# AIGeeksGroup/UniVid

Measured on AMD Instinct MI355X. Metric: denoise_steps_per_sec, higher is better.
Workload: dtype bf16

## Files before the change

include/univid_hip.h:

```cpp
#ifndef UNIVID_HIP_H
#define UNIVID_HIP_H
#include <stdint.h>
#ifdef __cplusplus
extern "C" {
#endif

int uv_version(void);
const char* uv_build_id(void);
int uv_init(void);
const char* uv_last_error(void);
int uv_device_arch(char* buf, int len);
int uv_host_blocking_sync(int on);

#define UV_OPT_CONV_HALO 0
#define UV_OPT_GEMM_GM 1
#define UV_OPT_ATTN_CUT 2
int uv_set_option(int key, int value);
int uv_get_option(int key, int* value);
int uv_reset_options(void);

#define UV_EPI_BF16 0
#define UV_EPI_GELU_BF16 1
#define UV_EPI_F32_FROM_BF16 2
#define UV_EPI_RESID_F32 3
#define UV_EPI_GATE_RESID_F32 4
#define UV_EPI_BF16_T 5

int uv_gemm_bf16_nt(const void* A, long lda, const void* W, long ldw, const void* bias_bf16, int M, int N, int K,
                    int epilogue, void* out, long ldo, const float* gate, const int32_t* gate_tid, long gate_stride,
                    int tile_cfg, void* stream);

int uv_gemm_bf16_nt_ws(const void* A, long lda, const void* W, long ldw, const void* bias_bf16, int M, int N, int K,
                       int epilogue, void* out, long ldo, const float* gate, const int32_t* gate_tid, long gate_stride,
                       int tile_cfg, void* workspace, long workspace_bytes, void* stream);
long uv_gemm_splitk_ws_bytes(int M, int N, int K);

int uv_gemm_f16_nt(const void* A, long lda, const void* W, long ldw, const void* bias_f16, int M, int N, int K, int epilogue,
                   void* out, long ldo, const float* gate, const int32_t* gate_tid, long gate_stride, int tile_cfg, void* stream);

int uv_gemm_bf16_nt_ssq(const void* A, long lda, const void* W, long ldw, const void* bias_bf16, int M, int N, int K, void* out, long ldo,
                        float* ssq, long ld_ssq, int tile_cfg, void* stream);
int uv_rms_scale_from_ssq(const float* ssq, long ld_ssq, int M, int groups, int C, float eps, float* rs, void* stream);

int uv_lora_down_bf16(const void* x, long ldx, const void* A, long lda, const float* scale, int M, int K, int R, void* out, long ldo,
                      int Rpad, void* stream);


int uv_mx_quant_bf16(const void* x, long ldx, void* codes, long ldc, void* scales, long ld_s, int M, int K, void* stream);

int uv_gemm_mxfp8_nt(const void* A, long lda, const void* A_scale, long ld_as, const void* W, long ldw, const void* W_scale, long ld_ws,
// ... 101 lines not shown
```

univid_amd/_lib.py:

```python
import ctypes
import os

import torch

_HERE = os.path.dirname(os.path.abspath(__file__))
LIB_PATH = os.path.join(_HERE, "libunivid_hip.so")

_c = ctypes
_P, _L, _I, _F = _c.c_void_p, _c.c_long, _c.c_int, _c.c_float

SIGNATURES = {
    "uv_version": [],
    "uv_init": [],
    "uv_last_error": [],
    "uv_build_id": [],
    "uv_device_arch": [_c.c_char_p, _I],
    "uv_host_blocking_sync": [_I],
    "uv_set_option": [_I, _I],
    "uv_get_option": [_I, _c.POINTER(_I)],
    "uv_reset_options": [],
    "uv_gemm_bf16_nt": [_P, _L, _P, _L, _P, _I, _I, _I, _I, _P, _L, _P, _P, _L, _I, _P],
    "uv_gemm_bf16_nt_ws": [_P, _L, _P, _L, _P, _I, _I, _I, _I, _P, _L, _P, _P, _L, _I, _P, _L, _P],
    "uv_gemm_splitk_ws_bytes": [_I, _I, _I],
    "uv_gemm_f16_nt": [_P, _L, _P, _L, _P, _I, _I, _I, _I, _P, _L, _P, _P, _L, _I, _P],
    "uv_mx_quant_bf16": [_P, _L, _P, _L, _P, _L, _I, _I, _P],
    "uv_gemm_mxfp8_nt": [_P, _L, _P, _L, _P, _L, _P, _L, _P, _I, _I, _I, _I, _P, _L, _P, _P, _L, _P],
    "uv_gemm_f32_nt": [_P, _L, _P, _L, _P, _I, _I, _I, _P, _L, _P, _L, _P],
    "uv_gemm_bf16_nt_ssq": [_P, _L, _P, _L, _P, _I, _I, _I, _P, _L, _P, _L, _I, _P],
    "uv_rms_scale_from_ssq": [_P, _L, _I, _I, _I, _F, _P, _P],
    "uv_lora_down_bf16": [_P, _L, _P, _L, _P, _I, _I, _I, _P, _L, _I, _P],
    "uv_cast_f32_bf16_rows": [_P, _L, _P, _L, _I, _I, _P],
    "uv_flash_attn_bf16_qnorm": [_P, _L, _P, _L, _P, _L, _P, _L, _I, _I, _I, _I, _I, _F, _P, _P, _P],
    "uv_flash_attn_bf16": [_P, _L, _P, _L, _P, _L, _P, _L, _I, _I, _I, _I, _I, _F, _P],
    "uv_flash_attn_f16": [_P, _L, _P, _L, _P, _L, _P, _L, _I, _I, _I, _I, _I, _F, _P],
    "uv_flash_attn_kernel_name": [_I, _I, _L, _L, _I, _c.c_char_p, _I],
    "uv_flash_attn_plan": [_I, _I, _I, _I, _I, _L, _L, _I, _c.c_char_p, _I, _c.POINTER(_I), _c.POINTER(_I), _c.POINTER(_I)],
    "uv_transpose_16": [_P, _L, _P, _L, _I, _I, _I, _P],
    "uv_cast_f32_to16": [_P, _P, _L, _I, _P],
# ... 31 lines not shown
    "uv_vae_split_f16": [_P, _L, _P, _L, _L, _I, _P, _P],
    "uv_split_weights_f16x3": [_P, _P, _L, _F, _P],
    "uv_split_weights_bf16x3": [_P, _P, _L, _P],
    "uv_split_weights_bf16x6": [_P, _P, _L, _P],
    "uv_vae_rms_silu": [_P, _L, _P, _P, _L, _L, _I, _I, _I, _P],
    "uv_softmax_rows_f32": [_P, _L, _I, _I, _F, _P],
    "uv_vae_dupup_add": [_P, _P, _I, _I, _I, _I, _I, _I, _I, _P],
    "uv_vae_avgdown_add": [_P, _P, _I, _I, _I, _I, _I, _I, _I, _P],
    "uv_vae_latent_in": [_P, _P, _P, _P, _L, _I, _L, _P],
    "uv_vae_latent_out": [_P, _L, _P, _P, _P, _I, _L, _P],
    "uv_vae_video_in": [_P, _P, _L, _I, _I, _I, _I, _I, _P],
    "uv_vae_video_out": [_P, _L, _P, _I, _I, _I, _I, _I, _P],
}
_RESTYPE = {"uv_last_error": _c.c_char_p, "uv_build_id": _c.c_char_p, "uv_gemm_splitk_ws_bytes": _L}

OPT_CONV_HALO, OPT_GEMM_GM, OPT_ATTN_CUT = range(3)
EPI_BF16, EPI_GELU_BF16, EPI_F32_FROM_BF16, EPI_RESID_F32, EPI_GATE_RESID_F32, EPI_BF16_T = range(6)

_lib = None
_inited = set()


class UnividHipError(RuntimeError):
    pass


def load(path=None):
    global _lib
    if _lib is not None:
        return _lib
    path = path or LIB_PATH
    if not os.path.exists(path):
# ... 136 lines not shown
    idx = torch.cuda.current_device() if dev.index is None else dev.index
    lib = load()
    with torch.cuda.device(idx):
        if lib.uv_host_blocking_sync(1 if on else 0) != 0:
            raise UnividHipError(lib.uv_last_error().decode())


def gemm_splitk_ws_bytes(M, N, K, device=None):
    dev = torch.device("cuda" if device is None else device)
    idx = torch.cuda.current_device() if dev.index is None else dev.index
    lib = init(idx)
    with torch.cuda.device(idx):
        return int(lib.uv_gemm_splitk_ws_bytes(int(M), int(N), int(K)))


def gemm_bf16(a, w, bias, out, epi, M=None, gate=None, gate_tid=None, tile_cfg=0, ws=None):
    f16 = a.dtype == torch.float16
    _chk(a, torch.float16 if f16 else torch.bfloat16, "gemm_bf16.a")
    _chk(w, a.dtype, "gemm_bf16.w")
    M = a.shape[0] if M is None else M
    N, K = w.shape
    if ws is not None and not f16:
        _chk(ws, torch.uint8, "gemm_bf16.ws")
        call("uv_gemm_bf16_nt_ws", ptr(a), a.stride(0), ptr(w), w.stride(0), ptr(bias), M, N, K, epi, ptr(out), out.stride(0),
             ptr(gate), ptr(gate_tid), 0 if gate is None else gate.stride(0), tile_cfg, ptr(ws), ws.numel(), stream_ptr(), flops=2 * M * N * K)
        return out
    call("uv_gemm_f16_nt" if f16 else "uv_gemm_bf16_nt", ptr(a), a.stride(0), ptr(w), w.stride(0), ptr(bias), M, N, K, epi, ptr(out), out.stride(0),
         ptr(gate), ptr(gate_tid), 0 if gate is None else gate.stride(0), tile_cfg, stream_ptr(), flops=2 * M * N * K)
    return out

# ... 162 lines not shown
```

univid_amd/csrc/capi.hip:

```cpp
#include "common.h"
#include <stdarg.h>
#include <stdio.h>
#include <atomic>

static thread_local char g_err[512] = "";

void uv_set_error(const char* fmt, ...) {
    va_list ap;
    va_start(ap, fmt);
    vsnprintf(g_err, sizeof(g_err), fmt, ap);
    va_end(ap);
}

extern "C" const char* uv_last_error(void) { return g_err; }

extern "C" int uv_version(void) { return 200; }

#ifndef UV_BUILD_ID
#define UV_BUILD_ID "unstamped"
#endif
extern "C" const char* uv_build_id(void) { return UV_BUILD_ID; }

static std::atomic<int> g_opt[UV_OPT_COUNT] = {{-1}, {0}, {0}};
static const int kOptDefault[UV_OPT_COUNT] = {-1, 0, 0};
int uv_option(int key) { return g_opt[key].load(std::memory_order_relaxed); }

extern "C" int uv_set_option(int key, int value) {
    UV_CHECK_ARG(key >= 0 && key < UV_OPT_COUNT, "uv_set_option: unknown key %d", key);
    if (key == UV_OPT_CONV_HALO) UV_CHECK_ARG(value >= -1 && value <= 1, "uv_set_option(UV_OPT_CONV_HALO): value %d not in {-1, 0, 1}", value);
    if (key == UV_OPT_GEMM_GM) UV_CHECK_ARG(value >= 0 && value <= 64, "uv_set_option(UV_OPT_GEMM_GM): value %d not in 0..64", value);
    if (key == UV_OPT_ATTN_CUT) UV_CHECK_ARG(value >= 0 && value <= 4096, "uv_set_option(UV_OPT_ATTN_CUT): value %d not in 0..4096", value);
    g_opt[key].store(value, std::memory_order_relaxed);
    return 0;
}

extern "C" int uv_get_option(int key, int* value) {
    UV_CHECK_ARG(key >= 0 && key < UV_OPT_COUNT && value, "uv_get_option: unknown key %d or null result pointer", key);
    *value = uv_option(key);
    return 0;
}

extern "C" int uv_reset_options(void) {
    for (int i = 0; i < UV_OPT_COUNT; ++i) g_opt[i].store(kOptDefault[i], std::memory_order_relaxed);
    return 0;
}
// ... 37 lines not shown
```

univid_amd/csrc/common.h:

```cpp
#pragma once
#include <hip/hip_runtime.h>
#include <stdint.h>
#include <mutex>

typedef uint16_t bf16_t;

typedef __attribute__((ext_vector_type(8))) __bf16 bf16x8;
typedef __attribute__((ext_vector_type(4))) __bf16 bf16x4;
typedef __attribute__((ext_vector_type(4))) float f32x4;
typedef __attribute__((ext_vector_type(16))) float f32x16;
typedef __attribute__((ext_vector_type(4))) uint32_t u32x4;
typedef __attribute__((ext_vector_type(2))) uint32_t u32x2;

#define UV_WAVE 64

#define UV_MAX_DEV 16
static inline int uv_cur_dev() {
    int d = 0;
    (void)hipGetDevice(&d);
    return (unsigned)d < UV_MAX_DEV ? d : 0;
}
#define UV_ONCE_PER_DEVICE(...)                                                      \
    do {                                                                             \
        static std::once_flag uv_once_[UV_MAX_DEV];                                  \
// ... 68 lines not shown
__device__ __forceinline__ f32x2 gelu_tanh_f32x2(f32x2 x) {
    const f32x2 kA = {-2.3022081986f, -2.3022081986f}, kB = {-0.1029432396f, -0.1029432396f}, one = {1.0f, 1.0f};
    const f32x2 q = __builtin_elementwise_fma(x * x, kB, kA);
    const f32x2 t = x * q;
    const f32x2 e = {__builtin_amdgcn_exp2f(t[0]), __builtin_amdgcn_exp2f(t[1])};
    const f32x2 d = one + e;
    const f32x2 c = {__builtin_amdgcn_rcpf(d[0]), __builtin_amdgcn_rcpf(d[1])};
    return x * c;
}

__device__ __forceinline__ float silu_f32(float x) { return x / (1.0f + expf(-x)); }

#define UV_OPT_CONV_HALO 0
#define UV_OPT_GEMM_GM 1
#define UV_OPT_ATTN_CUT 2
#define UV_OPT_COUNT 3
int uv_option(int key);

extern "C" const char* uv_last_error(void);
void uv_set_error(const char* fmt, ...);

#define UV_CHECK_ARG(cond, ...)            \
    do {                                   \
        if (!(cond)) {                     \
            uv_set_error(__VA_ARGS__);     \
            return -1;                     \
        }                                  \
    } while (0)

#define UV_CHECK_LAUNCH(name)                                                     \
    do {                                                                          \
// ... 7 lines not shown
```

univid_amd/csrc/gemm_bf16.hip:

```cpp
#include "gemm_bf16_kernels.h"
#include <limits.h>

int uv_gemm_diag_launch(const GemmArgs& a, int epilogue, int tile_cfg, hipStream_t s);

struct GemmWs { void* p = nullptr; long bytes = 0; };

enum GemmKernel {
    GK_PERSIST,
    GK_PINGPONG,
    GK_RING128,
    GK_T128,
    GK_T256,
    GK_T256x192,
    GK_SPLITK4,
    GK_SPLITK2,
    GK_DIAG,
};
struct GemmStep { GemmKernel kernel; int m0, rows; };
struct GemmPlan { int n; GemmStep step[2]; };

static long whole_rounds_cut(int M, int N, int ncus) {
    const long tiles_n = (N + 255) / 256, tiles_m = (M + 255) / 256;
    const long rounds = tiles_m * tiles_n / ncus;
    return rounds * ncus / tiles_n * 256;
}
static long persistent_cut(int M, int N, int ncus, bool* short_round) {
    const long tiles = (long)((M + 255) / 256) * (N / 256);
    const long rounds = tiles / ncus, rest = tiles - rounds * ncus;
    *short_round = rounds >= 1 && rest > 0 && rest * 100 < 45 * ncus;
    return *short_round ? whole_rounds_cut(M, N, ncus) : (long)(M / 256) * 256;
}

static GemmPlan plan_gemm(int M, int N, int K, int epilogue, long ldo, int tile_cfg, bool F16, int ncus, long ws_bytes, bool ws_aligned) {
    auto whole = [&](GemmKernel k) { return GemmPlan{1, {{k, 0, M}}}; };
    auto cut_at = [&](long cut, GemmKernel main, GemmKernel strip) {
        return cut <= 0 || cut >= M ? whole(main) : GemmPlan{2, {{main, 0, (int)cut}, {strip, (int)cut, M - (int)cut}}};
    };
    switch (tile_cfg) {
        case 0: break;
        case 1: return whole(GK_T128);
        case 5: return whole(GK_T256);
        case 6: return whole(GK_T256x192);
        case 7: return whole(GK_PINGPONG);
        case 8: return cut_at(whole_rounds_cut(M, N, ncus), GK_PINGPONG, GK_RING128);
        case 9: return cut_at(whole_rounds_cut(M, N, ncus), GK_T256, GK_RING128);
        case 12: return whole(GK_RING128);
        case 17: return whole(GK_PERSIST);
        case 18: {
            const long tm = (long)(M / 256) * 256;
            return cut_at(tm > 0 && tm < M ? tm : whole_rounds_cut(M, N, ncus), GK_PERSIST, GK_RING128);
        }
        case 19: return whole(GK_SPLITK4);
        case 20: return whole(GK_SPLITK2);
        default: return whole(GK_DIAG);
    }
    if (M >= 2048 && N >= 1024 && N % 256 == 0 && K % 128 == 0 && K >= 384 &&
        (ldo % 8 == 0 || epilogue == UV_EPI_BF16_T || (epilogue >= UV_EPI_F32_FROM_BF16 && epilogue != UV_EPI_BF16_SSQ))) {
        bool short_round = false;
        const long cut = persistent_cut(M, N, ncus, &short_round);
        if (cut / 256 * (N / 256) < 2L * ncus || (epilogue == UV_EPI_BF16_T && ldo % 8 != 0))
            return short_round ? cut_at(whole_rounds_cut(M, N, ncus), GK_PINGPONG, GK_RING128) : whole(GK_PINGPONG);
        const int rows = M - (int)cut;
        const long strip_tiles = (long)((rows + 255) / 256) * (N / 256);
        const bool splitk = !F16 && (epilogue == UV_EPI_BF16 || epilogue == UV_EPI_RESID_F32 || epilogue == UV_EPI_GATE_RESID_F32) &&
                            K >= 8192 && K % 512 == 0 && strip_tiles * 4 <= ncus && ws_aligned && ws_bytes >= splitk_ws_bytes(rows, N, 4);
        return cut_at(cut, GK_PERSIST, splitk ? GK_SPLITK4 : GK_RING128);
    }
    if (M < 2048 || N < 1024) {
        if (M >= 4096 && N >= 512 && N % 256 == 0 && K % 128 == 0 && K >= 256 && ldo % 8 == 0 && M % 256 == 0 &&
            2L * (M / 256) * (N / 256) >= ncus)
            return whole(GK_PINGPONG);
        const long t128 = (long)((M + 127) / 128) * ((N + 127) / 128);
        return whole(t128 <= 2 * ncus ? GK_RING128 : GK_T128);
    }
    const long tm = (M + 255) / 256;
    const long t256 = tm * ((N + 255) / 256), t192 = tm * ((N + 191) / 192);
    const double c256 = (double)((t256 + 255) / 256) * 1.00, c192 = (double)((t192 + 255) / 256) * 0.78;
    return whole(!F16 && N % 192 == 0 && c192 < c256 && K <= 4096 && epilogue != UV_EPI_BF16_SSQ ? GK_T256x192 : GK_T256);
}

static GemmArgs rows_of(const GemmArgs& a, int epilogue, long m0, int rows) {
    GemmArgs r = a;
    r.M = rows;
    r.A = a.A + m0 * a.lda;
    if (a.gate_tid) r.gate_tid = a.gate_tid + m0;
    if (a.ssq) r.ssq = a.ssq + m0 * a.ld_ssq;
    if (epilogue == UV_EPI_BF16_T) r.out = (bf16_t*)a.out + m0;
    else if (epilogue == UV_EPI_BF16 || epilogue == UV_EPI_GELU_BF16 || epilogue == UV_EPI_BF16_SSQ) r.out = (bf16_t*)a.out + m0 * a.ldo;
    else r.out = (float*)a.out + m0 * a.ldo;
    return r;
}

template <bool F16>
static int launch_step(GemmKernel kernel, const GemmArgs& a, int epilogue, int tile_cfg, hipStream_t s, const GemmWs& ws) {
    switch (kernel) {
        case GK_PERSIST:
            UV_CHECK_ARG(a.K % 128 == 0 && a.K >= 384, "uv_gemm_bf16_nt: tile_cfg 17 needs K %% 128 == 0 and K >= 384 (K=%d)", a.K);
            return launch_8ph_persist<F16>(a, epilogue, s);
        case GK_PINGPONG:
            UV_CHECK_ARG(a.K % 128 == 0 && a.K >= 256, "uv_gemm_bf16_nt: tile_cfg 7 needs K %% 128 == 0 and K >= 256 (K=%d)", a.K);
            return launch_8ph<5, F16>(a, epilogue, s);
        case GK_RING128: return launch_cfg<128, 128, 4, 2, 4, F16>(a, epilogue, s);
        case GK_T128: return launch_cfg<128, 128, 2, 2, 2, F16>(a, epilogue, s);
        case GK_T256: return launch_cfg<256, 256, 4, 4, 2, F16>(a, epilogue, s);
        case GK_T256x192: if constexpr (!F16) return launch_cfg<256, 192, 4, 4>(a, epilogue, s); break;
        case GK_SPLITK4: if constexpr (!F16) return launch_8ph_splitk<4, false>(a, epilogue, s, ws.p, ws.bytes); break;
        case GK_SPLITK2: if constexpr (!F16) return launch_8ph_splitk<2, false>(a, epilogue, s, ws.p, ws.bytes); break;
        case GK_DIAG: if constexpr (!F16) return uv_gemm_diag_launch(a, epilogue, tile_cfg, s); break;
    }
    uv_set_error("uv_gemm_f16_nt: tile_cfg %d is not built for fp16 operands", tile_cfg);
    return -1;
}

// ... 6 lines not shown
    UV_CHECK_ARG(K % UV_BK == 0, "uv_gemm_bf16_nt: K=%d must be a multiple of %d", K, UV_BK);
    UV_CHECK_ARG(N % 16 == 0, "uv_gemm_bf16_nt: N=%d must be a multiple of 16", N);
    UV_CHECK_ARG(lda % 8 == 0 && ldw % 8 == 0, "uv_gemm_bf16_nt: lda/ldw must be multiples of 8 elements");
    UV_CHECK_ARG(((uintptr_t)A & 15) == 0 && ((uintptr_t)W & 15) == 0 && ((uintptr_t)out & 15) == 0,
                 "uv_gemm_bf16_nt: pointers must be 16-byte aligned");
    UV_CHECK_ARG(ldo % 4 == 0, "uv_gemm_bf16_nt: ldo must be a multiple of 4 elements");
    if (epilogue == UV_EPI_GATE_RESID_F32)
        UV_CHECK_ARG(gate && gate_stride % 4 == 0, "uv_gemm_bf16_nt: gate table required (stride %% 4 == 0)");
    GemmArgs a;
    a.A = (const bf16_t*)A; a.W = (const bf16_t*)W; a.bias = (const bf16_t*)bias_bf16;
    a.out = out; a.gate = gate; a.gate_tid = gate_tid;
    a.lda = lda; a.ldw = ldw; a.ldo = ldo; a.gate_stride = gate_stride;
    a.M = M; a.N = N; a.K = K; a.tiles_m = a.tiles_n = 0;
    a.ssq = ssq; a.ld_ssq = ld_ssq;
    a.ws_slab = nullptr; a.ws_cnt = nullptr; a.gm = 0;
    if (epilogue == UV_EPI_BF16_SSQ)
        UV_CHECK_ARG(ssq && N % 32 == 0 && ld_ssq >= N / 32 && ldo % 8 == 0, "uv_gemm_bf16_nt_ssq: needs N %% 32 == 0, ld_ssq >= N / 32, ldo %% 8 == 0 (N=%d ld_ssq=%ld ldo=%ld)", N, ld_ssq, ldo);
    a.zeros = uv_zero_page();
    UV_CHECK_ARG(a.zeros, "uv_gemm_bf16_nt: zero page missing (call uv_init)");
    const GemmPlan plan = plan_gemm(M, N, K, epilogue, ldo, tile_cfg, F16, uv_num_cus(), ws.p ? ws.bytes : 0, ((uintptr_t)ws.p & 255) == 0);
    for (int i = 0; i < plan.n; ++i) {
        const GemmStep& st = plan.step[i];
        const int rc = launch_step<F16>(st.kernel, rows_of(a, epilogue, st.m0, st.rows), epilogue, tile_cfg, (hipStream_t)stream, ws);
        if (rc) return rc;
    }
    return 0;
}

extern "C" int uv_gemm_bf16_nt(const void* A, long lda, const void* W, long ldw, const void* bias_bf16,
                               int M, int N, int K, int epilogue, void* out, long ldo,
                               const float* gate, const int32_t* gate_tid, long gate_stride,
                               int tile_cfg, void* stream) {
    return gemm_entry<false>(A, lda, W, ldw, bias_bf16, M, N, K, epilogue, out, ldo, gate, gate_tid, gate_stride, tile_cfg, stream);
}

extern "C" int uv_gemm_bf16_nt_ws(const void* A, long lda, const void* W, long ldw, const void* bias_bf16,
                                  int M, int N, int K, int epilogue, void* out, long ldo,
                                  const float* gate, const int32_t* gate_tid, long gate_stride,
                                  int tile_cfg, void* workspace, long workspace_bytes, void* stream) {
    UV_CHECK_ARG(workspace_bytes >= 0 && (workspace || workspace_bytes == 0), "uv_gemm_bf16_nt_ws: bad workspace");
    GemmWs ws;
    ws.p = workspace; ws.bytes = workspace_bytes;
    return gemm_entry<false>(A, lda, W, ldw, bias_bf16, M, N, K, epilogue, out, ldo, gate, gate_tid, gate_stride, tile_cfg, stream, nullptr, 0, ws);
}

extern "C" long uv_gemm_splitk_ws_bytes(int M, int N, int K) {
    const GemmPlan plan = plan_gemm(M, N, K, UV_EPI_RESID_F32, N, 0, false, uv_num_cus(), LONG_MAX, true);
    const GemmStep& strip = plan.step[plan.n - 1];
    return strip.kernel == GK_SPLITK4 ? splitk_ws_bytes(strip.rows, N, 4) : 0;
}

extern "C" int uv_gemm_bf16_nt_ssq(const void* A, long lda, const void* W, long ldw, const void* bias_bf16, int M, int N, int K,
                                   void* out, long ldo, float* ssq, long ld_ssq, int tile_cfg, void* stream) {
    return gemm_entry<false>(A, lda, W, ldw, bias_bf16, M, N, K, UV_EPI_BF16_SSQ, out, ldo, nullptr, nullptr, 0, tile_cfg, stream, ssq, ld_ssq);
}

extern "C" int uv_gemm_f16_nt(const void* A, long lda, const void* W, long ldw, const void* bias_f16,
                              int M, int N, int K, int epilogue, void* out, long ldo,
                              const float* gate, const int32_t* gate_tid, long gate_stride,
                              int tile_cfg, void* stream) {
    UV_CHECK_ARG(tile_cfg == 0, "uv_gemm_f16_nt: only tile_cfg 0 (automatic) is built for fp16 operands");
    return gemm_entry<true>(A, lda, W, ldw, bias_f16, M, N, K, epilogue, out, ldo, gate, gate_tid, gate_stride, tile_cfg, stream);
}
```

univid_amd/csrc/gemm_bf16_kernels.h:

```cpp
#pragma once
#include "common.h"
#include <stdlib.h>
#include <type_traits>

const float* uv_zero_page();

#define UV_BK 64

enum {
    UV_EPI_BF16 = 0,
    UV_EPI_GELU_BF16 = 1,
    UV_EPI_F32_FROM_BF16 = 2,
    UV_EPI_RESID_F32 = 3,
    UV_EPI_GATE_RESID_F32 = 4,
    UV_EPI_BF16_T = 5,
    UV_EPI_BF16_SSQ = 6,
};

struct GemmArgs {
    const bf16_t* A;
    const bf16_t* W;
    const bf16_t* bias;
    void* out;
    const float* gate;
    const int32_t* gate_tid;
    const float* zeros;
    long lda, ldw, ldo, gate_stride;
    int M, N, K;
    int tiles_m, tiles_n;
    int gm;
    float* ssq;
    long ld_ssq;
    float* ws_slab;
    int* ws_cnt;
};

typedef __attribute__((address_space(3))) void lds_void;

__device__ __forceinline__ void glds16(const void* g, lds_void* l) {
    __builtin_amdgcn_global_load_lds(g, l, 16, 0, 0);
}

template <int EPI, bool F16 = false, bool FULL = false>
__device__ __forceinline__ void epi_frag(const GemmArgs& p, int mb, int nb, const f32x4& a, int frow, int fq) {
    if (EPI != UV_EPI_BF16_T) {
        const int m = mb + frow, n = nb + 4 * fq;
        if (!FULL && (m >= p.M || n >= p.N)) return;
        float v[4];
#pragma unroll
// ... 164 lines not shown
        const int m = mb[f] + frow, n = nb[f] + 4 * fq;
        float v[4];
        v[0] = acc[f][0] + in16<F16>((bf16_t)(bb[slot][0] & 0xffff));
        v[1] = acc[f][1] + in16<F16>((bf16_t)(bb[slot][0] >> 16));
        v[2] = acc[f][2] + in16<F16>((bf16_t)(bb[slot][1] & 0xffff));
        v[3] = acc[f][3] + in16<F16>((bf16_t)(bb[slot][1] >> 16));
        f32x4 x = xb[slot];
#pragma unroll
        for (int e = 0; e < 4; ++e)
            x[e] = GATE ? __fadd_rn(x[e], __fmul_rn(round16<F16>(v[e]), gb[slot][e])) : __fadd_rn(x[e], round16<F16>(v[e]));
        if (m < p.M && n < p.N) *(f32x4*)((float*)p.out + (long)m * p.ldo + n) = x;
        if (f + D < NF) issue(f + D, slot);
    }
}

template <int BM, int BN, int WM, int WN, int EPI, int NS = 2, bool F16 = false>
__global__ __launch_bounds__(WM* WN * 64) void gemm_bf16_nt_kernel(GemmArgs p) {
    constexpr int NW = WM * WN;
    constexpr int NT = NW * 64;
    constexpr int TM = BM / WM / 16;
    constexpr int TN = BN / WN / 16;
    constexpr int A_BYTES = BM * 128;
    constexpr int W_BYTES = BN * 128;
    constexpr int STAGE_BYTES = A_BYTES + W_BYTES;
    constexpr int A_INSTR = (BM / 8 + NW - 1) / NW;
    constexpr int W_INSTR = (BN / 8 + NW - 1) / NW;
    static_assert(BM % 8 == 0 && BN % 8 == 0 && (BM / WM) % 16 == 0 && (BN / WN) % 16 == 0, "tile/wave mismatch");
    constexpr bool TRANS = (EPI == UV_EPI_BF16_T);

    extern __shared__ __attribute__((aligned(16))) char smem[];

    const int tid = threadIdx.x;
    const int lane = tid & 63;
    const int wave = __builtin_amdgcn_readfirstlane(tid >> 6);
    const int wm = wave / WN, wn = wave % WN;

    const int nblk = p.tiles_m * p.tiles_n;
    int bid = blockIdx.x;
    {
        const int q = nblk >> 3, r = nblk & 7, xcd = bid & 7, idx = bid >> 3;
        bid = (xcd < r ? xcd * (q + 1) : r * (q + 1) + (xcd - r) * q) + idx;
    }
    constexpr int GM = 4;
    const int group_sz = GM * p.tiles_n;
    const int group = bid / group_sz;
    const int first_m = group * GM;
    const int gm = min(GM, p.tiles_m - first_m);
    const int in_group = bid - group * group_sz;
    const int tile_m = first_m + in_group % gm;
    const int tile_n = in_group / gm;
    const int m0 = tile_m * BM, n0 = tile_n * BN;

    const int srow = lane >> 3;
    const int pchunk = lane & 7;
    const bf16_t* a_src[A_INSTR];
    const bf16_t* w_src[W_INSTR];
#pragma unroll
    for (int i = 0; i < A_INSTR; ++i) {
        const int row = (i * NW + wave) * 8 + srow;
        const int c = pchunk ^ ((row >> 1) & 7);
        const int gr = min(m0 + row, p.M - 1);
        a_src[i] = p.A + (long)gr * p.lda + c * 8;
    }
#pragma unroll
    for (int i = 0; i < W_INSTR; ++i) {
        const int row = (i * NW + wave) * 8 + srow;
// ... 107 lines not shown
        epi_rmw_pipe<EPI, NF, (NF >= 8 ? 4 : 2), F16>(p, mb, nb, av, frow, fq);
    } else if constexpr (EPI == UV_EPI_BF16_SSQ) {
        static_assert(TN % 2 == 0 && (BN / WN) % 32 == 0, "UV_EPI_BF16_SSQ needs whole 32-column groups per wave");
#pragma unroll
        for (int j = 0; j < TM; ++j)
#pragma unroll
            for (int i = 0; i < TN; i += 2)
                epi_pair_ssq<F16>(p, m0 + wm * (BM / WM) + j * 16, n0 + wn * (BN / WN) + i * 16, acc[i][j], acc[i + 1][j], frow, fq);
    } else {
#pragma unroll
        for (int j = 0; j < TM; ++j)
#pragma unroll
            for (int i = 0; i < TN; ++i)
                epi_frag<EPI, F16>(p, m0 + wm * (BM / WM) + j * 16, n0 + wn * (BN / WN) + i * 16, acc[i][j], frow, fq);
    }
}


template <int EPI, bool F16>
__device__ __forceinline__ void epi_rmw_rows_lds(const GemmArgs& p, char* smem, const f32x4 (&acc)[2][2][2][4], int m0, int n0,
                                                 int wave, int lane) {
    static_assert(EPI == UV_EPI_RESID_F32 || EPI == UV_EPI_GATE_RESID_F32, "rmw epilogues only");
    constexpr bool GATE = EPI == UV_EPI_GATE_RESID_F32;
    constexpr int D = 8;
    const int wr = wave >> 2, wc = wave & 3;
    const int frow = lane & 15, fq = lane >> 4;
    float bv[2][2][4];
#pragma unroll
    for (int hn = 0; hn < 2; ++hn)
#pragma unroll
// ... 314 lines not shown
                for (int hn = 0; hn < 2; ++hn)
                    epi_pair_ssq<F16>(p, m0 + hm * 128 + wr * 64 + j * 16, n0 + hn * 128 + wc * 32, acc[hn][hm][0][j], acc[hn][hm][1][j], frow, fq);
    } else {
#pragma unroll
        for (int hm = 0; hm < 2; ++hm)
#pragma unroll
            for (int j = 0; j < 4; ++j)
#pragma unroll
                for (int hn = 0; hn < 2; ++hn)
#pragma unroll
                    for (int i = 0; i < 2; ++i)
                        epi_frag<EPI, F16>(p, m0 + hm * 128 + wr * 64 + j * 16, n0 + hn * 128 + wc * 32 + i * 16, acc[hn][hm][i][j], frow, fq);
    }
}

template <int EPI, bool F16 = false>
__global__ __launch_bounds__(512) void gemm_bf16_8ph_persist_kernel(GemmArgs p) {
    constexpr bool TRANS = (EPI == UV_EPI_BF16_T);
    constexpr bool RMW = (EPI == UV_EPI_RESID_F32 || EPI == UV_EPI_GATE_RESID_F32);
    constexpr int VAR = 5;
    constexpr int HALF = 16384;
    constexpr int BUF = 4 * HALF;
    extern __shared__ __attribute__((aligned(16))) char smem[];

    const int tid = threadIdx.x;
    const int lane = tid & 63;
    const int wave = __builtin_amdgcn_readfirstlane(tid >> 6);
    const int wr = wave >> 2, wc = wave & 3;

    const int nblk = p.tiles_m * p.tiles_n;
    const int G = gridDim.x >> 3;
    int first, cnt;
    {
        const int q = nblk >> 3, r = nblk & 7, xcd = blockIdx.x & 7;
        first = xcd < r ? xcd * (q + 1) : r * (q + 1) + (xcd - r) * q;
        cnt = q + (xcd < r ? 1 : 0);
    }
    int cur = blockIdx.x >> 3;
    if (cur >= cnt) return;
    const int GM = p.gm;
    const int group_sz = GM * p.tiles_n;
    auto origin = [&](int bid, int& m0, int& n0) {
        const int group = bid / group_sz;
        const int first_m = group * GM;
        const int gm = min(GM, p.tiles_m - first_m);
        const int in_group = bid - group * group_sz;
        m0 = (first_m + in_group % gm) * 256;
        n0 = (in_group / gm) * 256;
    };
    int m0, n0;
    origin(first + cur, m0, n0);

    const int srow = lane >> 3, pchunk = lane & 7;
    const bf16_t* a_src[2][2];
// ... 90 lines not shown
                        for (int i = 0; i < 2; ++i)
                            epi_pair16_T<F16>(p, m0 + hm * 128 + wr * 64 + j * 16, n0 + hn * 128 + wc * 32 + i * 16, acc[hn][hm][i][j], acc[hn][hm][i][j + 1], frow, fq);
        } else {
#pragma unroll
            for (int hm = 0; hm < 2; ++hm)
#pragma unroll
                for (int j = 0; j < 4; ++j)
#pragma unroll
                    for (int hn = 0; hn < 2; ++hn)
#pragma unroll
                        for (int i = 0; i < 2; ++i)
                            epi_frag<EPI, F16, true>(p, m0 + hm * 128 + wr * 64 + j * 16, n0 + hn * 128 + wc * 32 + i * 16, acc[hn][hm][i][j], frow, fq);
        }
        if (!has_next) break;
        m0 = m1; n0 = n1; cur = nxt;
    }
    asm volatile("s_waitcnt vmcnt(0)" ::: "memory");
}


template <void (*KERN)(GemmArgs)>
static int launch_kernel(dim3 grid, dim3 block, size_t lds, hipStream_t stream, const GemmArgs& a, const char* who) {
    UV_ONCE_PER_DEVICE(hipFuncSetAttribute((const void*)KERN, hipFuncAttributeMaxDynamicSharedMemorySize, (int)lds));
    hipLaunchKernelGGL(KERN, grid, block, lds, stream, a);
    UV_CHECK_LAUNCH(who);
    return 0;
}

constexpr unsigned UV_EPIS_ALL = 0x7f;
constexpr bool epi_in(unsigned epis, int e) { return e >= 0 && e < 32 && (epis >> e & 1) != 0; }
// ... 40 lines not shown
    constexpr unsigned EPIS = 1u << UV_EPI_BF16 | 1u << UV_EPI_RESID_F32 | 1u << UV_EPI_GATE_RESID_F32;
    UV_CHECK_ARG(epi_in(EPIS, epi),
                 "uv_gemm_bf16_nt_ws: the split-K strip is built for the bf16 and the residual epilogues (0, 3, 4), not %d", epi);
    a.ws_cnt = (int*)ws;
    a.ws_slab = (float*)((char*)ws + 4096);
    if (hipMemsetAsync(a.ws_cnt, 0, (size_t)tiles * sizeof(int), stream) != hipSuccess) {
        uv_set_error("uv_gemm_bf16_nt_ws: hipMemsetAsync of the tile counters failed");
        return -1;
    }
    const dim3 grid(8 * ((tiles * SK + 7) / 8));
    return launch_epi<EPIS>(epi, [&](auto e) {
        return launch_kernel<gemm_bf16_8ph_kernel<decltype(e)::value, 5, F16, SK>>(grid, 512, 128 * 1024, stream, a, "uv_gemm_bf16_nt_ws");
    });
}

template <bool F16 = false>
static int launch_8ph_persist(const GemmArgs& a0, int epi, hipStream_t stream) {
    GemmArgs a = a0;
    UV_CHECK_ARG(a.M % 256 == 0 && a.N % 256 == 0, "uv_gemm_bf16_nt: the persistent kernel needs whole 256x256 tiles (M=%d N=%d)", a.M, a.N);
    UV_CHECK_ARG(a.ldo % 8 == 0 || (epi != UV_EPI_BF16_T && epi != UV_EPI_BF16 && epi != UV_EPI_GELU_BF16 && epi != UV_EPI_BF16_SSQ),
                 "uv_gemm_bf16_nt: the persistent kernel stores 16 bytes per lane: ldo=%ld must be a multiple of 8 elements", a.ldo);
    a.tiles_m = a.M / 256;
    a.tiles_n = a.N / 256;
    a.gm = (a.N <= 4096 && a.K <= 4096) ? 8 : (a.K >= 8192 ? 2 : 4);
    if (const int gm = uv_option(UV_OPT_GEMM_GM); gm > 0) a.gm = gm;
    const int tiles = a.tiles_m * a.tiles_n;
    int wgs = uv_num_cus() & ~7;
    if (wgs > tiles) wgs = tiles & ~7;
    UV_CHECK_ARG(wgs >= 8, "uv_gemm_bf16_nt: too few tiles (%d) for the persistent kernel", tiles);
    const dim3 grid(wgs);
    return launch_epi(epi, [&](auto e) {
        return launch_kernel<gemm_bf16_8ph_persist_kernel<decltype(e)::value, F16>>(grid, 512, 128 * 1024, stream, a, "uv_gemm_bf16_nt");
    });
}

template <int BM, int BN, int WM, int WN, int NS = 2, bool F16 = false>
static int launch_cfg(const GemmArgs& a0, int epi, hipStream_t stream) {
    GemmArgs a = a0;
    a.tiles_m = (a.M + BM - 1) / BM;
    a.tiles_n = (a.N + BN - 1) / BN;
    constexpr bool SSQ = (BN / WN) % 32 == 0;
    UV_CHECK_ARG(SSQ || epi != UV_EPI_BF16_SSQ, "uv_gemm_bf16_nt_ssq: this tile shape has no whole 32-column groups per wave");
    const dim3 grid(a.tiles_m * a.tiles_n);
    return launch_epi<SSQ ? UV_EPIS_ALL : UV_EPIS_ALL & ~(1u << UV_EPI_BF16_SSQ)>(epi, [&](auto e) {
        return launch_kernel<gemm_bf16_nt_kernel<BM, BN, WM, WN, decltype(e)::value, NS, F16>>(grid, WM * WN * 64, NS * (BM + BN) * 128, stream, a, "uv_gemm_bf16_nt");
    });
}
// ... 1 lines not shown
```

Measured before the change: 3.946.

## Fold the leftover row strip into the persistent GEMM kernel as 128x128 tail tiles

```diff
diff --git a/include/univid_hip.h b/include/univid_hip.h
--- a/include/univid_hip.h
+++ b/include/univid_hip.h
@@ -15,6 +15,7 @@
 #define UV_OPT_CONV_HALO 0
 #define UV_OPT_GEMM_GM 1
 #define UV_OPT_ATTN_CUT 2
+#define UV_OPT_GEMM_TAIL 3
 int uv_set_option(int key, int value);
 int uv_get_option(int key, int* value);
 int uv_reset_options(void);
@@ -34,6 +35,9 @@
                        int epilogue, void* out, long ldo, const float* gate, const int32_t* gate_tid, long gate_stride,
                        int tile_cfg, void* workspace, long workspace_bytes, void* stream);
 long uv_gemm_splitk_ws_bytes(int M, int N, int K);
+
+int uv_gemm_plan(int M, int N, int K, int epilogue, long ldo, int tile_cfg, int f16, int ncus, int* steps, int* n_steps);
+int uv_gemm_tail_tiles(int tail_rows, int N, int grid, int wg, int* tile_m, int* tile_n, int cap, int* count);
 
 int uv_gemm_f16_nt(const void* A, long lda, const void* W, long ldw, const void* bias_f16, int M, int N, int K, int epilogue,
                    void* out, long ldo, const float* gate, const int32_t* gate_tid, long gate_stride, int tile_cfg, void* stream);
diff --git a/univid_amd/_lib.py b/univid_amd/_lib.py
--- a/univid_amd/_lib.py
+++ b/univid_amd/_lib.py
@@ -22,6 +22,8 @@
     "uv_gemm_bf16_nt": [_P, _L, _P, _L, _P, _I, _I, _I, _I, _P, _L, _P, _P, _L, _I, _P],
     "uv_gemm_bf16_nt_ws": [_P, _L, _P, _L, _P, _I, _I, _I, _I, _P, _L, _P, _P, _L, _I, _P, _L, _P],
     "uv_gemm_splitk_ws_bytes": [_I, _I, _I],
+    "uv_gemm_plan": [_I, _I, _I, _I, _L, _I, _I, _I, _c.POINTER(_I), _c.POINTER(_I)],
+    "uv_gemm_tail_tiles": [_I, _I, _I, _I, _c.POINTER(_I), _c.POINTER(_I), _I, _c.POINTER(_I)],
     "uv_gemm_f16_nt": [_P, _L, _P, _L, _P, _I, _I, _I, _I, _P, _L, _P, _P, _L, _I, _P],
     "uv_mx_quant_bf16": [_P, _L, _P, _L, _P, _L, _I, _I, _P],
     "uv_gemm_mxfp8_nt": [_P, _L, _P, _L, _P, _L, _P, _L, _P, _I, _I, _I, _I, _P, _L, _P, _P, _L, _P],
@@ -83,8 +85,8 @@
 }
 _RESTYPE = {"uv_last_error": _c.c_char_p, "uv_build_id": _c.c_char_p, "uv_gemm_splitk_ws_bytes": _L}
 
-OPT_CONV_HALO, OPT_GEMM_GM, OPT_ATTN_CUT = range(3)
-EPI_BF16, EPI_GELU_BF16, EPI_F32_FROM_BF16, EPI_RESID_F32, EPI_GATE_RESID_F32, EPI_BF16_T = range(6)
+OPT_CONV_HALO, OPT_GEMM_GM, OPT_ATTN_CUT, OPT_GEMM_TAIL = range(4)
+EPI_BF16, EPI_GELU_BF16, EPI_F32_FROM_BF16, EPI_RESID_F32, EPI_GATE_RESID_F32, EPI_BF16_T, EPI_BF16_SSQ = range(7)
 
 _lib = None
 _inited = set()
@@ -251,6 +253,26 @@
         return int(lib.uv_gemm_splitk_ws_bytes(int(M), int(N), int(K)))
 
 
+GK_PERSIST, GK_PINGPONG, GK_RING128 = range(3)
+
+
+def gemm_plan(M, N, K, epi=EPI_BF16, ldo=None, tile_cfg=0, f16=False, ncus=0):
+    steps, n = (_I * 10)(), _I(0)
+    lib = load()
+    if lib.uv_gemm_plan(int(M), int(N), int(K), int(epi), int(N if ldo is None else ldo), int(tile_cfg), int(f16), int(ncus), steps, ctypes.byref(n)) != 0:
+        raise UnividHipError(lib.uv_last_error().decode())
+    return [tuple(steps[5 * i:5 * i + 5]) for i in range(n.value)]
+
+
+def gemm_tail_tiles(tail_rows, N, grid, wg):
+    cap = (tail_rows + 127) // 128 * (N // 128) + 1
+    tm, tn, n = (_I * cap)(), (_I * cap)(), _I(0)
+    lib = load()
+    if lib.uv_gemm_tail_tiles(int(tail_rows), int(N), int(grid), int(wg), tm, tn, cap, ctypes.byref(n)) != 0:
+        raise UnividHipError(lib.uv_last_error().decode())
+    return [(tm[i], tn[i]) for i in range(n.value)]
+
+
 def gemm_bf16(a, w, bias, out, epi, M=None, gate=None, gate_tid=None, tile_cfg=0, ws=None):
     f16 = a.dtype == torch.float16
     _chk(a, torch.float16 if f16 else torch.bfloat16, "gemm_bf16.a")
diff --git a/univid_amd/csrc/capi.hip b/univid_amd/csrc/capi.hip
--- a/univid_amd/csrc/capi.hip
+++ b/univid_amd/csrc/capi.hip
@@ -21,14 +21,15 @@
 #endif
 extern "C" const char* uv_build_id(void) { return UV_BUILD_ID; }
 
-static std::atomic<int> g_opt[UV_OPT_COUNT] = {{-1}, {0}, {0}};
-static const int kOptDefault[UV_OPT_COUNT] = {-1, 0, 0};
+static std::atomic<int> g_opt[UV_OPT_COUNT] = {{-1}, {0}, {0}, {0}};
+static const int kOptDefault[UV_OPT_COUNT] = {-1, 0, 0, 0};
 int uv_option(int key) { return g_opt[key].load(std::memory_order_relaxed); }
 
 extern "C" int uv_set_option(int key, int value) {
     UV_CHECK_ARG(key >= 0 && key < UV_OPT_COUNT, "uv_set_option: unknown key %d", key);
     if (key == UV_OPT_CONV_HALO) UV_CHECK_ARG(value >= -1 && value <= 1, "uv_set_option(UV_OPT_CONV_HALO): value %d not in {-1, 0, 1}", value);
     if (key == UV_OPT_GEMM_GM) UV_CHECK_ARG(value >= 0 && value <= 64, "uv_set_option(UV_OPT_GEMM_GM): value %d not in 0..64", value);
+    if (key == UV_OPT_GEMM_TAIL) UV_CHECK_ARG(value >= 0 && value <= 2, "uv_set_option(UV_OPT_GEMM_TAIL): value %d not in {0, 1, 2}", value);
     if (key == UV_OPT_ATTN_CUT) UV_CHECK_ARG(value >= 0 && value <= 4096, "uv_set_option(UV_OPT_ATTN_CUT): value %d not in 0..4096", value);
     g_opt[key].store(value, std::memory_order_relaxed);
     return 0;
diff --git a/univid_amd/csrc/common.h b/univid_amd/csrc/common.h
--- a/univid_amd/csrc/common.h
+++ b/univid_amd/csrc/common.h
@@ -106,7 +106,8 @@
 #define UV_OPT_CONV_HALO 0
 #define UV_OPT_GEMM_GM 1
 #define UV_OPT_ATTN_CUT 2
-#define UV_OPT_COUNT 3
+#define UV_OPT_GEMM_TAIL 3
+#define UV_OPT_COUNT 4
 int uv_option(int key);
 
 extern "C" const char* uv_last_error(void);
diff --git a/univid_amd/csrc/gemm_bf16.hip b/univid_amd/csrc/gemm_bf16.hip
--- a/univid_amd/csrc/gemm_bf16.hip
+++ b/univid_amd/csrc/gemm_bf16.hip
@@ -16,7 +16,7 @@
     GK_SPLITK2,
     GK_DIAG,
 };
-struct GemmStep { GemmKernel kernel; int m0, rows; };
+struct GemmStep { GemmKernel kernel; int m0, rows, tail; };
 struct GemmPlan { int n; GemmStep step[2]; };
 
 static long whole_rounds_cut(int M, int N, int ncus) {
@@ -31,10 +31,11 @@
     return *short_round ? whole_rounds_cut(M, N, ncus) : (long)(M / 256) * 256;
 }
 
-static GemmPlan plan_gemm(int M, int N, int K, int epilogue, long ldo, int tile_cfg, bool F16, int ncus, long ws_bytes, bool ws_aligned) {
-    auto whole = [&](GemmKernel k) { return GemmPlan{1, {{k, 0, M}}}; };
+static GemmPlan plan_gemm(int M, int N, int K, int epilogue, long ldo, int tile_cfg, bool F16, int ncus, long ws_bytes, bool ws_aligned,
+                          bool two_launch) {
+    auto whole = [&](GemmKernel k) { return GemmPlan{1, {{k, 0, M, 0}}}; };
     auto cut_at = [&](long cut, GemmKernel main, GemmKernel strip) {
-        return cut <= 0 || cut >= M ? whole(main) : GemmPlan{2, {{main, 0, (int)cut}, {strip, (int)cut, M - (int)cut}}};
+        return cut <= 0 || cut >= M ? whole(main) : GemmPlan{2, {{main, 0, (int)cut, 0}, {strip, (int)cut, M - (int)cut, 0}}};
     };
     switch (tile_cfg) {
         case 0: break;
@@ -64,7 +65,8 @@
         const long strip_tiles = (long)((rows + 255) / 256) * (N / 256);
         const bool splitk = !F16 && (epilogue == UV_EPI_BF16 || epilogue == UV_EPI_RESID_F32 || epilogue == UV_EPI_GATE_RESID_F32) &&
                             K >= 8192 && K % 512 == 0 && strip_tiles * 4 <= ncus && ws_aligned && ws_bytes >= splitk_ws_bytes(rows, N, 4);
-        return cut_at(cut, GK_PERSIST, splitk ? GK_SPLITK4 : GK_RING128);
+        if (splitk || two_launch || cut <= 0 || cut >= M) return cut_at(cut, GK_PERSIST, splitk ? GK_SPLITK4 : GK_RING128);
+        return GemmPlan{1, {{GK_PERSIST, 0, M, rows}}};
     }
     if (M < 2048 || N < 1024) {
         if (M >= 4096 && N >= 512 && N % 256 == 0 && K % 128 == 0 && K >= 256 && ldo % 8 == 0 && M % 256 == 0 &&
@@ -92,11 +94,11 @@
 }
 
 template <bool F16>
-static int launch_step(GemmKernel kernel, const GemmArgs& a, int epilogue, int tile_cfg, hipStream_t s, const GemmWs& ws) {
+static int launch_step(GemmKernel kernel, const GemmArgs& a, int tail, int epilogue, int tile_cfg, hipStream_t s, const GemmWs& ws) {
     switch (kernel) {
         case GK_PERSIST:
             UV_CHECK_ARG(a.K % 128 == 0 && a.K >= 384, "uv_gemm_bf16_nt: tile_cfg 17 needs K %% 128 == 0 and K >= 384 (K=%d)", a.K);
-            return launch_8ph_persist<F16>(a, epilogue, s);
+            return launch_8ph_persist<F16>(a, epilogue, s, tail);
         case GK_PINGPONG:
             UV_CHECK_ARG(a.K % 128 == 0 && a.K >= 256, "uv_gemm_bf16_nt: tile_cfg 7 needs K %% 128 == 0 and K >= 256 (K=%d)", a.K);
             return launch_8ph<5, F16>(a, epilogue, s);
@@ -133,14 +135,16 @@
     a.M = M; a.N = N; a.K = K; a.tiles_m = a.tiles_n = 0;
     a.ssq = ssq; a.ld_ssq = ld_ssq;
     a.ws_slab = nullptr; a.ws_cnt = nullptr; a.gm = 0;
+    a.tail_m0 = a.tail_rows = a.tail_fwd = 0;
     if (epilogue == UV_EPI_BF16_SSQ)
         UV_CHECK_ARG(ssq && N % 32 == 0 && ld_ssq >= N / 32 && ldo % 8 == 0, "uv_gemm_bf16_nt_ssq: needs N %% 32 == 0, ld_ssq >= N / 32, ldo %% 8 == 0 (N=%d ld_ssq=%ld ldo=%ld)", N, ld_ssq, ldo);
     a.zeros = uv_zero_page();
     UV_CHECK_ARG(a.zeros, "uv_gemm_bf16_nt: zero page missing (call uv_init)");
-    const GemmPlan plan = plan_gemm(M, N, K, epilogue, ldo, tile_cfg, F16, uv_num_cus(), ws.p ? ws.bytes : 0, ((uintptr_t)ws.p & 255) == 0);
+    const GemmPlan plan = plan_gemm(M, N, K, epilogue, ldo, tile_cfg, F16, uv_num_cus(), ws.p ? ws.bytes : 0, ((uintptr_t)ws.p & 255) == 0,
+                                    uv_option(UV_OPT_GEMM_TAIL) == 1);
     for (int i = 0; i < plan.n; ++i) {
         const GemmStep& st = plan.step[i];
-        const int rc = launch_step<F16>(st.kernel, rows_of(a, epilogue, st.m0, st.rows), epilogue, tile_cfg, (hipStream_t)stream, ws);
+        const int rc = launch_step<F16>(st.kernel, rows_of(a, epilogue, st.m0, st.rows), st.tail, epilogue, tile_cfg, (hipStream_t)stream, ws);
         if (rc) return rc;
     }
     return 0;
@@ -164,9 +168,33 @@
 }
 
 extern "C" long uv_gemm_splitk_ws_bytes(int M, int N, int K) {
-    const GemmPlan plan = plan_gemm(M, N, K, UV_EPI_RESID_F32, N, 0, false, uv_num_cus(), LONG_MAX, true);
+    const GemmPlan plan = plan_gemm(M, N, K, UV_EPI_RESID_F32, N, 0, false, uv_num_cus(), LONG_MAX, true, uv_option(UV_OPT_GEMM_TAIL) == 1);
     const GemmStep& strip = plan.step[plan.n - 1];
     return strip.kernel == GK_SPLITK4 ? splitk_ws_bytes(strip.rows, N, 4) : 0;
+}
+
+extern "C" int uv_gemm_plan(int M, int N, int K, int epilogue, long ldo, int tile_cfg, int f16, int ncus, int* steps, int* n_steps) {
+    UV_CHECK_ARG(M > 0 && N > 0 && K > 0 && ncus >= 0 && steps && n_steps, "uv_gemm_plan: bad shape M=%d N=%d K=%d, CU count %d or null result pointer", M, N, K, ncus);
+    const GemmPlan plan = plan_gemm(M, N, K, epilogue, ldo, tile_cfg, f16 != 0, ncus ? ncus : uv_num_cus(), 0, true, uv_option(UV_OPT_GEMM_TAIL) == 1);
+    for (int i = 0; i < plan.n; ++i) {
+        const GemmStep& st = plan.step[i];
+        steps[5 * i] = st.kernel; steps[5 * i + 1] = st.m0; steps[5 * i + 2] = st.rows; steps[5 * i + 3] = st.tail;
+        steps[5 * i + 4] = st.kernel == GK_PERSIST ? persist_grid(ncus ? ncus : uv_num_cus(), (long)((st.rows - st.tail) / 256) * (N / 256)) : 0;
+    }
+    *n_steps = plan.n;
+    return 0;
+}
+
+extern "C" int uv_gemm_tail_tiles(int tail_rows, int N, int grid, int wg, int* tile_m, int* tile_n, int cap, int* count) {
+    UV_CHECK_ARG(tail_rows >= 0 && N > 0 && N % 128 == 0 && grid >= 8 && grid % 8 == 0 && wg >= 0 && wg < grid && tile_m && tile_n && cap >= 0 && count,
+                 "uv_gemm_tail_tiles: bad arguments (tail_rows=%d N=%d grid=%d wg=%d)", tail_rows, N, grid, wg);
+    const int ttm = (tail_rows + 127) >> 7, ttn = N >> 7, G = grid >> 3;
+    int tfirst, tcnt, n = 0;
+    xcd_range(ttm * ttn, wg & 7, tfirst, tcnt);
+    for (int tt = tail_slot(wg >> 3, G, uv_option(UV_OPT_GEMM_TAIL) == 2); tt < tcnt; tt += G, ++n)
+        if (n < cap) walk4_tile(tfirst + tt, ttm, ttn, tile_m[n], tile_n[n]);
+    *count = n;
+    return 0;
 }
 
 extern "C" int uv_gemm_bf16_nt_ssq(const void* A, long lda, const void* W, long ldw, const void* bias_bf16, int M, int N, int K,
diff --git a/univid_amd/csrc/gemm_bf16_kernels.h b/univid_amd/csrc/gemm_bf16_kernels.h
--- a/univid_amd/csrc/gemm_bf16_kernels.h
+++ b/univid_amd/csrc/gemm_bf16_kernels.h
@@ -33,6 +33,8 @@
     long ld_ssq;
     float* ws_slab;
     int* ws_cnt;
+    int tail_m0, tail_rows;
+    int tail_fwd;
 };
 
 typedef __attribute__((address_space(3))) void lds_void;
@@ -227,8 +229,8 @@
     }
 }
 
-template <int BM, int BN, int WM, int WN, int EPI, int NS = 2, bool F16 = false>
-__global__ __launch_bounds__(WM* WN * 64) void gemm_bf16_nt_kernel(GemmArgs p) {
+template <int BM, int BN, int WM, int WN, int EPI, int NS, bool F16>
+__device__ __forceinline__ void gemm_nt_tile(const GemmArgs& p, char* smem, int m0, int n0, int tid) {
     constexpr int NW = WM * WN;
     constexpr int NT = NW * 64;
     constexpr int TM = BM / WM / 16;
@@ -241,28 +243,10 @@
     static_assert(BM % 8 == 0 && BN % 8 == 0 && (BM / WM) % 16 == 0 && (BN / WN) % 16 == 0, "tile/wave mismatch");
     constexpr bool TRANS = (EPI == UV_EPI_BF16_T);
 
-    extern __shared__ __attribute__((aligned(16))) char smem[];
-
-    const int tid = threadIdx.x;
+
     const int lane = tid & 63;
     const int wave = __builtin_amdgcn_readfirstlane(tid >> 6);
     const int wm = wave / WN, wn = wave % WN;
-
-    const int nblk = p.tiles_m * p.tiles_n;
-    int bid = blockIdx.x;
-    {
-        const int q = nblk >> 3, r = nblk & 7, xcd = bid & 7, idx = bid >> 3;
-        bid = (xcd < r ? xcd * (q + 1) : r * (q + 1) + (xcd - r) * q) + idx;
-    }
-    constexpr int GM = 4;
-    const int group_sz = GM * p.tiles_n;
-    const int group = bid / group_sz;
-    const int first_m = group * GM;
-    const int gm = min(GM, p.tiles_m - first_m);
-    const int in_group = bid - group * group_sz;
-    const int tile_m = first_m + in_group % gm;
-    const int tile_n = in_group / gm;
-    const int m0 = tile_m * BM, n0 = tile_n * BN;
 
     const int srow = lane >> 3;
     const int pchunk = lane & 7;
@@ -400,6 +384,34 @@
             for (int i = 0; i < TN; ++i)
                 epi_frag<EPI, F16>(p, m0 + wm * (BM / WM) + j * 16, n0 + wn * (BN / WN) + i * 16, acc[i][j], frow, fq);
     }
+}
+
+__host__ __device__ __forceinline__ void walk4_tile(int t, int tiles_m, int tiles_n, int& tile_m, int& tile_n) {
+    constexpr int GM = 4;
+    const int group_sz = GM * tiles_n;
+    const int group = t / group_sz;
+    const int first_m = group * GM;
+    const int gm = tiles_m - first_m < GM ? tiles_m - first_m : GM;
+    const int in_group = t - group * group_sz;
+    tile_m = first_m + in_group % gm;
+    tile_n = in_group / gm;
+}
+
+__host__ __device__ __forceinline__ void xcd_range(int n, int xcd, int& first, int& cnt) {
+    const int q = n >> 3, r = n & 7;
+    first = xcd < r ? xcd * (q + 1) : r * (q + 1) + (xcd - r) * q;
+    cnt = q + (xcd < r ? 1 : 0);
+}
+
+__host__ __device__ __forceinline__ int tail_slot(int idx, int G, int fwd) { return fwd ? idx : G - 1 - idx; }
+
+template <int BM, int BN, int WM, int WN, int EPI, int NS = 2, bool F16 = false>
+__global__ __launch_bounds__(WM* WN * 64) void gemm_bf16_nt_kernel(GemmArgs p) {
+    extern __shared__ __attribute__((aligned(16))) char smem[];
+    int first, cnt, tile_m, tile_n;
+    xcd_range(p.tiles_m * p.tiles_n, blockIdx.x & 7, first, cnt);
+    walk4_tile(first + (blockIdx.x >> 3), p.tiles_m, p.tiles_n, tile_m, tile_n);
+    gemm_nt_tile<BM, BN, WM, WN, EPI, NS, F16>(p, smem, tile_m * BM, tile_n * BN, threadIdx.x);
 }
 
 
@@ -744,7 +756,7 @@
     }
 }
 
-template <int EPI, bool F16 = false>
+template <int EPI, bool F16 = false, bool TAIL = false>
 __global__ __launch_bounds__(512) void gemm_bf16_8ph_persist_kernel(GemmArgs p) {
     constexpr bool TRANS = (EPI == UV_EPI_BF16_T);
     constexpr bool RMW = (EPI == UV_EPI_RESID_F32 || EPI == UV_EPI_GATE_RESID_F32);
@@ -758,16 +770,13 @@
     const int wave = __builtin_amdgcn_readfirstlane(tid >> 6);
     const int wr = wave >> 2, wc = wave & 3;
 
-    const int nblk = p.tiles_m * p.tiles_n;
     const int G = gridDim.x >> 3;
     int first, cnt;
-    {
-        const int q = nblk >> 3, r = nblk & 7, xcd = blockIdx.x & 7;
-        first = xcd < r ? xcd * (q + 1) : r * (q + 1) + (xcd - r) * q;
-        cnt = q + (xcd < r ? 1 : 0);
-    }
+    xcd_range(p.tiles_m * p.tiles_n, blockIdx.x & 7, first, cnt);
     int cur = blockIdx.x >> 3;
-    if (cur >= cnt) return;
+    if constexpr (!TAIL) {
+        if (cur >= cnt) return;
+    }
     const int GM = p.gm;
     const int group_sz = GM * p.tiles_n;
     auto origin = [&](int bid, int& m0, int& n0) {
@@ -888,6 +897,20 @@
         }
         if (!has_next) break;
         m0 = m1; n0 = n1; cur = nxt;
+    }
+    if constexpr (TAIL) {
+        const int ttm = (p.tail_rows + 127) >> 7, ttn = p.N >> 7;
+        int tfirst, tcnt;
+        xcd_range(ttm * ttn, blockIdx.x & 7, tfirst, tcnt);
+        for (int tt = tail_slot(blockIdx.x >> 3, G, p.tail_fwd); tt < tcnt; tt += G) {
+            int tile_m, tile_n;
+            walk4_tile(tfirst + tt, ttm, ttn, tile_m, tile_n);
+            asm volatile("s_waitcnt lgkmcnt(0)" ::: "memory");
+            __builtin_amdgcn_s_barrier();
+            int ttid = (wave << 6) | (int)__builtin_amdgcn_mbcnt_hi(~0u, __builtin_amdgcn_mbcnt_lo(~0u, 0u));
+            asm volatile("" : "+v"(ttid));
+            gemm_nt_tile<128, 128, 4, 2, EPI, 4, F16>(p, smem, p.tail_m0 + tile_m * 128, tile_n * 128, ttid);
+        }
     }
     asm volatile("s_waitcnt vmcnt(0)" ::: "memory");
 }
@@ -958,23 +981,34 @@
     });
 }
 
+static inline int persist_grid(int ncus, long tiles) {
+    int wgs = ncus & ~7;
+    if (wgs > tiles) wgs = (int)tiles & ~7;
+    return wgs;
+}
+
 template <bool F16 = false>
-static int launch_8ph_persist(const GemmArgs& a0, int epi, hipStream_t stream) {
+static int launch_8ph_persist(const GemmArgs& a0, int epi, hipStream_t stream, int tail_rows = 0) {
     GemmArgs a = a0;
-    UV_CHECK_ARG(a.M % 256 == 0 && a.N % 256 == 0, "uv_gemm_bf16_nt: the persistent kernel needs whole 256x256 tiles (M=%d N=%d)", a.M, a.N);
+    const int main_rows = a.M - tail_rows;
+    UV_CHECK_ARG(tail_rows >= 0 && main_rows > 0 && main_rows % 256 == 0 && a.N % 256 == 0,
+                 "uv_gemm_bf16_nt: the persistent kernel needs whole 256x256 tiles (M=%d less %d tail rows, N=%d)", a.M, tail_rows, a.N);
     UV_CHECK_ARG(a.ldo % 8 == 0 || (epi != UV_EPI_BF16_T && epi != UV_EPI_BF16 && epi != UV_EPI_GELU_BF16 && epi != UV_EPI_BF16_SSQ),
                  "uv_gemm_bf16_nt: the persistent kernel stores 16 bytes per lane: ldo=%ld must be a multiple of 8 elements", a.ldo);
-    a.tiles_m = a.M / 256;
+    a.tiles_m = main_rows / 256;
     a.tiles_n = a.N / 256;
+    a.tail_m0 = main_rows;
+    a.tail_rows = tail_rows;
+    a.tail_fwd = uv_option(UV_OPT_GEMM_TAIL) == 2;
     a.gm = (a.N <= 4096 && a.K <= 4096) ? 8 : (a.K >= 8192 ? 2 : 4);
     if (const int gm = uv_option(UV_OPT_GEMM_GM); gm > 0) a.gm = gm;
     const int tiles = a.tiles_m * a.tiles_n;
-    int wgs = uv_num_cus() & ~7;
-    if (wgs > tiles) wgs = tiles & ~7;
+    const int wgs = persist_grid(uv_num_cus(), tiles);
     UV_CHECK_ARG(wgs >= 8, "uv_gemm_bf16_nt: too few tiles (%d) for the persistent kernel", tiles);
     const dim3 grid(wgs);
     return launch_epi(epi, [&](auto e) {
-        return launch_kernel<gemm_bf16_8ph_persist_kernel<decltype(e)::value, F16>>(grid, 512, 128 * 1024, stream, a, "uv_gemm_bf16_nt");
+        if (tail_rows > 0) return launch_kernel<gemm_bf16_8ph_persist_kernel<decltype(e)::value, F16, true>>(grid, 512, 128 * 1024, stream, a, "uv_gemm_bf16_nt");
+        return launch_kernel<gemm_bf16_8ph_persist_kernel<decltype(e)::value, F16, false>>(grid, 512, 128 * 1024, stream, a, "uv_gemm_bf16_nt");
     });
 }
 
```

Measured after the change: 3.958 (median of 6 runs). No clear change (+0.3%).
